# ALVI-Labs/frankenstein

Hardware: AMD Instinct MI355X
Metric: neural frames/sec (train fwd+bwd+AdamW, whole job) (higher is better)
Workload: dtype bf16; 1 GPU; brainformer-small (6L d=384 6x64 heads, N=6144 tokens) + 2-block perceiver, L1 head; fwd+bwd+clip+AdamW; per_gpu_batch=32, global_batch=32, frames_T=600, electrodes=256, parallelism=dp1, weights=random-init (seed 42)

## Files before the change

### frankenstein_amd/_lib.py

```python
from __future__ import annotations

import ctypes as C
from pathlib import Path

import os

LIB_PATH = Path(os.environ.get("FRANKEN_HIP_LIB") or Path(__file__).resolve().parent / "libfranken_hip.so")

FK_F32, FK_BF16 = 0, 1
MASK_NONE, MASK_CAUSAL, MASK_BLOCK_CAUSAL, MASK_PREFIX, MASK_KEYPAD, MASK_DENSE = 0, 1, 2, 3, 4, 5
NORM_LAYER, NORM_RMS = 0, 1
ATTN_Q_PRESCALED = 1
GEMV_GELU = 1
NT_RING2, NT_RING192, NT_RING128, NT_BIG, NT_GLDS4, NT_GLDS, NT_STAGED = range(7)
NT_LANE = 7
MLP_BWD_HIPCC, MLP_BWD_ASM = 0, 1
NT_ROUTE_F32 = -2
ATTN_FWD_GENERIC, ATTN_FWD_FEWQ, ATTN_FWD_PS, ATTN_FWD_ASM = range(4)
ATTN_DQ_GENERIC, ATTN_DQ_FEWQ, ATTN_DQ_PS, ATTN_DQ_ASM = range(4)
ATTN_DKDV_GENERIC, ATTN_DKDV_PS, ATTN_DKDV_ASM, ATTN_DKDVW_ASM = range(4)

_p, _i64, _int, _f32, _f64, _sz, _u32 = C.c_void_p, C.c_int64, C.c_int, C.c_float, C.c_double, C.c_size_t, C.c_uint32

SIGNATURES = {
    "fk_version": (_int, []),
    "fk_last_error": (C.c_char_p, []),
    "fk_gemm_nt": (_int, [_p, _i64, _p, _i64, _p, _i64, _i64, _i64, _i64, _p, _p, _i64, _i64, _int, _int, _p]),
    "fk_gemv_nt": (_int, [_p, _i64, _p, _i64, _p, _i64, _i64, _i64, _i64, _p, _p, _i64, _p, _p, _f32, _int, _int, _int, _p]),
    "fk_gemm_nt_rope": (_int, [_p, _i64, _p, _i64, _p, _i64, _i64, _i64, _i64, _p, _p, _i64, _i64, _i64, _i64, _i64, _i64, _i64, _int, _p]),
    "fk_gemm_nt_swiglu": (_int, [_p, _i64, _p, _i64, _p, _i64, _p, _i64, _i64, _i64, _i64, _int, _p]),
    "fk_gemm_nt_dswiglu": (_int, [_p, _i64, _p, _i64, _p, _i64, _p, _i64, _i64, _i64, _i64, _int, _p]),
    "fk_mlp_bwd_fused": (_int, [_p, _i64, _p, _i64, _p, _i64, _p, _i64, _p, _i64, _p, _i64, _i64, _i64, _i64, _int, _p]),
    "fk_gemm_nt_route": (_int, [_i64, _i64, _i64, _int, _int, _int, _int]),
    "fk_gemm_nt_rope_route": (_int, [_i64] * 6 + [_int] + [_i64] * 5 + [_int, _int]),
    "fk_gemm_nt_swiglu_route": (_int, [_i64] * 7 + [_int, _int]),
    "fk_mlp_bwd_fused_route": (_int, [_i64, _i64]),
    "fk_gemm_tn_route": (_int, [_i64, _i64, _i64, _int, _p, _p]),
    "fk_gemm_tn_workspace_bytes": (_sz, [_i64, _i64, _i64, _int]),
    "fk_gemm_tn": (_int, [_p, _i64, _p, _i64, _p, _i64, _i64, _i64, _i64, _int, _int, _p, _sz, _p]),
    "fk_gemm_tn_swiglu": (_int, [_p, _i64, _p, _i64, _p, _p, _i64, _i64, _i64, _i64, _int, _p, _sz, _p]),
    "fk_colsum_workspace_bytes": (_sz, [_i64, _i64]),
    "fk_colsum": (_int, [_p, _i64, _p, _i64, _i64, _int, _int, _p, _sz, _p]),
    "fk_attn_fwd": (_int, [_p, _p, _p, _p, _p] + [_i64] * 13 + [_int, _i64, _i64, _i64, _p, _p, _f32, _int, _int, _p]),
    "fk_attn_bwd": (_int, [_p] * 10 + [_i64] * 13 + [_int, _i64, _i64, _i64, _p, _p, _f32, _p, _i64, _i64, _int, _int, _p]),
    "fk_attn_fwd_dropout": (_int, [_p, _p, _p, _p, _p] + [_i64] * 13 + [_int, _i64, _i64, _i64, _p, _p, _f32, _int, _f32, _p, _u32, _int, _p]),
    "fk_attn_bwd_dropout": (_int, [_p] * 10 + [_i64] * 13 + [_int, _i64, _i64, _i64, _p, _p, _f32, _p, _i64, _i64, _int, _f32, _p, _u32, _int, _p]),
    "fk_attn_route": (_int, [_i64, _i64, _i64, _int, _int, _i64, _i64, _i64, _int, _int, _int, _p, _p, _p]),
    "fk_dropout": (_int, [_p, _p, _p, _i64, _f32, _p, _u32, _int, _p]),
    "fk_norm_fwd": (_int, [_p, _p, _p, _p, _p, _p, _i64, _i64, _f32, _int, _int, _p]),
    "fk_norm_bwd_workspace_bytes": (_sz, [_i64, _i64]),
    "fk_norm_bwd": (_int, [_p] * 9 + [_i64, _i64, _int, _int, _int, _p, _sz, _p]),
    "fk_rope": (_int, [_p, _i64, _i64, _i64, _i64, _i64, _p, _i64, _i64, _int, _int, _p]),
    "fk_patchify": (_int, [_p, _p, _i64, _i64, _i64, _i64, _i64, _int, _p]),
    "fk_swiglu_fwd": (_int, [_p, _p, _i64, _i64, _int, _p]),
    "fk_swiglu_bwd": (_int, [_p, _p, _p, _i64, _i64, _int, _p]),
    "fk_gelu_fwd": (_int, [_p, _p, _i64, _int, _p]),
    "fk_gelu_bwd": (_int, [_p, _p, _p, _i64, _int, _p]),
    "fk_cast_pack": (_int, [_p, _i64, _p, _i64, _i64, _i64, _int, _int, _p]),
    "fk_cast_pack_rows": (_int, [_p, _i64, _p, _i64, _i64, _i64, _int, _i64, _i64, _i64, _int, _p]),
    "fk_cast_pack_multi": (_int, [_p, _i64, _i64, _int, _p]),
    "fk_cast": (_int, [_p, _int, _p, _int, _i64, _p]),
    "fk_add": (_int, [_p, _p, _p, _i64, _int, _p]),
    "fk_gather_rows": (_int, [_p, _i64, _int, _p, _i64, _p, _i64, _int, _i64, _i64, _i64, _int, _p]),
# ... 141 lines not shown
```

### frankenstein_amd/csrc/gemm.hip

```cpp
#include <type_traits>

#include "fk_common.h"

namespace {

#ifndef FK_EPI_UNROLL
#define FK_EPI_UNROLL 1
#endif
#include "gemm_tile.h"

struct NtArgs {
  const void* A; const void* B; void* C;
  const void* bias; const void* res;
  int64_t lda, ldb, ldc, ldr, res_rows;
  int M, N, K, vec_epi;
  int mode;
  void* aux; int64_t ldaux;
  const float* rope_table; int64_t rope_bs; int rope_T, rope_off, rope_D, rope_cols;
  int rope_qcols; int64_t rope_qoff;
};

#ifndef FK_NT_STORES_GEMM
#define FK_NT_STORES_GEMM 1
#endif
// ... 1235 lines not shown
    for (; kt + TG_NS - 1 < nk; ++kt) step(Yes{}, Yes{}, Vm1{});
    if (kt + 2 < nk) { step(Yes{}, No{}, Vm1{}); ++kt; }
    if (kt + 1 < nk) step(Yes{}, No{}, Vm0{});
    step(No{}, No{}, Vm0{});
  }

  float* out = (p.nsplit > 1) ? p.ws + (int64_t)split * p.N1 * p.N2 : p.C;
  const int64_t ldo = (p.nsplit > 1) ? p.N2 : p.ldc;
  const bool accum = (p.nsplit == 1) && p.accumulate;
#pragma unroll
  for (int j = 0; j < NJ; ++j) {
    const int n = b0 + wn * WB + j * 32 + li;
#pragma unroll
    for (int i = 0; i < 3; ++i)
#pragma unroll
      for (int r = 0; r < 16; ++r) {
        const int m = a0 + wm * 96 + i * 32 + acc_row(r, lh);
        float* dst = out + (int64_t)m * ldo + n;
        *dst = accum ? (*dst + acc[i][j][r]) : acc[i][j][r];
      }
  }
}

template <bool IL>
__global__ __launch_bounds__(256) void reduce_slabs4_kernel(const float* ws, float* C, float* C1, int64_t ldc, int N1, int N2, int nsplit, int accumulate) {
  const int64_t total = (int64_t)N1 * N2, total4 = total >> 2;
  const int n2v = N2 >> 2;
  for (int64_t i = blockIdx.x * (int64_t)blockDim.x + threadIdx.x; i < total4; i += (int64_t)gridDim.x * blockDim.x) {
    const f32x4* src = reinterpret_cast<const f32x4*>(ws) + i;
    f32x4 s = {0.0f, 0.0f, 0.0f, 0.0f};
    int k = 0;
    for (; k + 8 <= nsplit; k += 8) {
      f32x4 v[8];
#pragma unroll
      for (int u = 0; u < 8; ++u) v[u] = src[(int64_t)(k + u) * total4];
#pragma unroll
      for (int u = 0; u < 8; ++u) s += v[u];
    }
    for (; k < nsplit; ++k) s += src[(int64_t)k * total4];
    int64_t r = i / n2v;
    float* base = C;
    if constexpr (IL) {
      if (r & 4) base = C1;
      r = (r >> 3) * 4 + (r & 3);
    }
    f32x4* dst = reinterpret_cast<f32x4*>(base + r * ldc + (i % n2v) * 4);
    if (accumulate) s += *dst;
    *dst = s;
  }
}
__global__ void reduce_slabs_kernel(const float* ws, float* C, int64_t ldc, int N1, int N2, int nsplit, int accumulate) {
  const int64_t total = (int64_t)N1 * N2;
  for (int64_t i = blockIdx.x * (int64_t)blockDim.x + threadIdx.x; i < total; i += (int64_t)gridDim.x * blockDim.x) {
    float s = 0.0f;
    for (int k = 0; k < nsplit; ++k) s += ws[k * total + i];
    float* dst = C + (i / N2) * ldc + (i % N2);
    *dst = accumulate ? (*dst + s) : s;
  }
}

template <typename T>
__global__ __launch_bounds__(256) void colsum_partial_kernel(const T* X, int64_t ld, float* part, int rows, int cols, int rows_per_blk) {
  constexpr int N = 16 / sizeof(T);
  __shared__ float red[256 * N];
  const int r0 = blockIdx.y * rows_per_blk, r1 = min(rows, r0 + rows_per_blk);
  const int cvt = (cols + N - 1) / N;
  {
    const int cv0 = blockIdx.x * 256;
    const int cvn = min(256, cvt - cv0), groups = 256 / cvn;
// ... 216 lines not shown

static int tn_plan(int64_t M, int64_t N1, int64_t N2, int dtype, int* nsplit, int64_t* rows_per_split) {
  const bool big = tn_big_ok(M, N1, N2, dtype);
  const int bkm = dtype == FK_BF16 ? 64 : 32;
  const int ns = big ? tn_big_splits(M, N1, N2) : tn_splits(M, N1, N2, bkm);
  if (nsplit) *nsplit = ns;
  if (rows_per_split) *rows_per_split = fk_cdiv(fk_cdiv(M, ns), bkm) * bkm;
  return big ? tn_big_tb(N1, N2) : 0;
}

int fk_gemm_tn_route(int64_t M, int64_t N1, int64_t N2, int dtype, int* nsplit, int64_t* rows_per_split) {
  FK_CHECK_ARG(dtype == FK_F32 || dtype == FK_BF16, "fk_gemm_tn_route: bad dtype %d", dtype);
  FK_CHECK_ARG(M > 0 && N1 > 0 && N2 > 0, "fk_gemm_tn_route: empty problem");
  return tn_plan(M, N1, N2, dtype, nsplit, rows_per_split);
}

size_t fk_gemm_tn_workspace_bytes(int64_t M, int64_t N1, int64_t N2, int dtype) {
  int ns;
  tn_plan(M, N1, N2, dtype, &ns, nullptr);
  return ns > 1 ? (size_t)ns * N1 * N2 * sizeof(float) : 0;
}

static int launch_tn(const void* A, int64_t lda, const void* B, int64_t ldb, float* C, float* C1, int64_t ldc, int64_t M, int64_t N1,
                     int64_t N2, int accumulate, int dtype, void* workspace, size_t workspace_bytes, void* stream) {
  FK_CHECK_ARG(dtype == FK_F32 || dtype == FK_BF16, "fk_gemm_tn: bad dtype %d", dtype);
  const int vec = dtype == FK_BF16 ? 8 : 4;
  FK_CHECK_ARG(M > 0 && N1 > 0 && N2 > 0, "fk_gemm_tn: empty problem");
  FK_CHECK_ARG(M < (1LL << 31) && N1 < (1LL << 31) && N2 < (1LL << 31), "fk_gemm_tn: dims must fit int32");
  FK_CHECK_ARG(N1 % vec == 0 && N2 % vec == 0 && lda % vec == 0 && ldb % vec == 0,
               "fk_gemm_tn: N1/N2/lda/ldb must be multiples of %d (N1=%lld N2=%lld)", vec, (long long)N1, (long long)N2);
  FK_CHECK_ARG(((uintptr_t)A & 15) == 0 && ((uintptr_t)B & 15) == 0, "fk_gemm_tn: A/B must be 16-byte aligned");
  int ns;
  int64_t rps;
  const int tb = tn_plan(M, N1, N2, dtype, &ns, &rps);
  const bool big = tb != 0;
  const size_t need = ns > 1 ? (size_t)ns * N1 * N2 * sizeof(float) : 0;
  FK_CHECK_ARG(workspace_bytes >= need && (need == 0 || workspace), "fk_gemm_tn: workspace too small (%zu < %zu)", workspace_bytes, need);
  if (C1)
    FK_CHECK_ARG(ns > 1 && N1 % 8 == 0 && N2 % 4 == 0 && ldc % 4 == 0 && (((uintptr_t)C | (uintptr_t)C1 | (uintptr_t)workspace) & 15) == 0,
                 "fk_gemm_tn_swiglu: needs a split plan (see fk_gemm_tn_route), N1 %% 8 == 0, N2 %% 4 == 0 and 16-byte aligned destinations");
  TnArgs p{A, B, C, (float*)workspace, lda, ldb, ldc, (int)M, (int)N1, (int)N2, (int)rps, ns, accumulate};
  dim3 grid((unsigned)(fk_cdiv(N1, BM) * fk_cdiv(N2, BN) * ns)), block(NTHREADS);
  hipStream_t s = (hipStream_t)stream;
  if (big) {
    dim3 bgrid((unsigned)((N1 / TG_A) * (N2 / tb) * ns));
    if (tb == 192) {
      constexpr int LDS192 = TG_NS * (TG_A_BYTES + TG_K * 512);
      fk_launch_lds<gemm_tn_big_kernel<192>>(bgrid, dim3(512), LDS192, s, p);
    } else {
      fk_launch_lds<gemm_tn_big_kernel<128>>(bgrid, dim3(512), TG_NS * TG_STAGE, s, p);
    }
  } else if (dtype == FK_BF16) hipLaunchKernelGGL((gemm_tn_kernel<bf16_t>), grid, block, 4 * TILE_BYTES, s, p);
  else hipLaunchKernelGGL((gemm_tn_kernel<float>), grid, block, 4 * TILE_BYTES, s, p);
  FK_CHECK_LAUNCH("fk_gemm_tn");
  if (ns > 1) {
    const int64_t total = N1 * N2;
    if (N2 % 4 == 0 && ldc % 4 == 0 && (((uintptr_t)C | (uintptr_t)workspace) & 15) == 0) {
      int nb = (int)fk_cdiv(total / 4, 256);
      if (nb > 2048) nb = 2048;
      if (C1) hipLaunchKernelGGL(reduce_slabs4_kernel<true>, dim3(nb), dim3(256), 0, s, (const float*)workspace, C, C1, ldc, (int)N1, (int)N2, ns, accumulate);
      else hipLaunchKernelGGL(reduce_slabs4_kernel<false>, dim3(nb), dim3(256), 0, s, (const float*)workspace, C, C1, ldc, (int)N1, (int)N2, ns, accumulate);
    } else {
      int nb = (int)fk_cdiv(total, 256);
      if (nb > 2048) nb = 2048;
      hipLaunchKernelGGL(reduce_slabs_kernel, dim3(nb), dim3(256), 0, s, (const float*)workspace, C, ldc, (int)N1, (int)N2, ns, accumulate);
    }
    FK_CHECK_LAUNCH("fk_gemm_tn(reduce)");
  }
  return FK_OK;
}

int fk_gemm_tn(const void* A, int64_t lda, const void* B, int64_t ldb, float* C, int64_t ldc, int64_t M, int64_t N1,
               int64_t N2, int accumulate, int dtype, void* workspace, size_t workspace_bytes, void* stream) {
  return launch_tn(A, lda, B, ldb, C, nullptr, ldc, M, N1, N2, accumulate, dtype, workspace, workspace_bytes, stream);
}

int fk_gemm_tn_swiglu(const void* A, int64_t lda, const void* B, int64_t ldb, float* d_up, float* d_gate, int64_t ldc, int64_t M,
                      int64_t H, int64_t N2, int dtype, void* workspace, size_t workspace_bytes, void* stream) {
  FK_CHECK_ARG(d_up && d_gate && H > 0 && H % 4 == 0, "fk_gemm_tn_swiglu: needs both destinations and H %% 4 == 0");
  return launch_tn(A, lda, B, ldb, d_up, d_gate, ldc, M, 2 * H, N2, 1, dtype, workspace, workspace_bytes, stream);
}

size_t fk_colsum_workspace_bytes(int64_t rows, int64_t cols) { return (size_t)colsum_blocks(rows) * cols * sizeof(float); }

int fk_colsum(const void* X, int64_t ld, float* out, int64_t rows, int64_t cols, int accumulate, int dtype,
              void* workspace, size_t workspace_bytes, void* stream) {
  FK_CHECK_ARG(dtype == FK_F32 || dtype == FK_BF16, "fk_colsum: bad dtype %d", dtype);
  FK_CHECK_ARG(rows > 0 && cols > 0 && rows < (1LL << 31) && cols < (1LL << 31), "fk_colsum: bad shape");
  const int nb = colsum_blocks(rows);
  FK_CHECK_ARG(workspace && workspace_bytes >= (size_t)nb * cols * sizeof(float), "fk_colsum: workspace too small");
  const int rpb = (int)fk_cdiv(rows, nb);
  hipStream_t s = (hipStream_t)stream;
  const int vec = dtype == FK_BF16 ? 8 : 4;
  if (cols % vec == 0 && ld % vec == 0 && ((uintptr_t)X & 15) == 0) {
    dim3 grid((unsigned)fk_cdiv(fk_cdiv(cols, vec), 256), (unsigned)nb), block(256);
    if (dtype == FK_BF16) hipLaunchKernelGGL(colsum_partial_kernel<bf16_t>, grid, block, 0, s, (const bf16_t*)X, ld, (float*)workspace, (int)rows, (int)cols, rpb);
    else hipLaunchKernelGGL(colsum_partial_kernel<float>, grid, block, 0, s, (const float*)X, ld, (float*)workspace, (int)rows, (int)cols, rpb);
  } else {
    dim3 grid((unsigned)fk_cdiv(cols, 256), (unsigned)nb), block(256);
    if (dtype == FK_BF16) hipLaunchKernelGGL(colsum_partial_scalar_kernel<bf16_t>, grid, block, 0, s, (const bf16_t*)X, ld, (float*)workspace, (int)rows, (int)cols, rpb);
    else hipLaunchKernelGGL(colsum_partial_scalar_kernel<float>, grid, block, 0, s, (const float*)X, ld, (float*)workspace, (int)rows, (int)cols, rpb);
  }
  FK_CHECK_LAUNCH("fk_colsum(partial)");
// ... 7 lines not shown
```

### frankenstein_amd/engine.py

```python
from __future__ import annotations

from typing import List, NamedTuple, Optional, Sequence, Tuple

import dataclasses
import math
import os
import weakref

import torch

from . import kernels as K
from .kernels import NO_MASK

Tensor = torch.Tensor

_COMPUTE_DTYPE = torch.bfloat16
_EPOCH = 0


def set_compute_dtype(dtype) -> None:
    global _COMPUTE_DTYPE
    if isinstance(dtype, str):
        dtype = {"bf16": torch.bfloat16, "bfloat16": torch.bfloat16, "fp32": torch.float32, "float32": torch.float32}[dtype]
    assert dtype in (torch.bfloat16, torch.float32)
# ... 8 lines not shown
    global _EPOCH
    _EPOCH += 1


_WGRAD_STREAM = None


def enable_wgrad_stream(on: bool = True):
    global _WGRAD_STREAM
    _WGRAD_STREAM = torch.cuda.Stream() if on else None
    return _WGRAD_STREAM


def wgrad_stream():
    return _WGRAD_STREAM


def _arena_grad(p: Tensor):
    g = p.grad
    return g if (g is not None and getattr(p, "_fk_arena", False) and g.is_contiguous()) else None


def wgrad_path(in_arena: Sequence[bool], swiglu_interleaved: bool = False, slab_ok: bool = False, adjacent: bool = False,
               requires_grad: Optional[Sequence[bool]] = None) -> str:
    if requires_grad is not None and not any(requires_grad):
        return "skip"
    if not all(in_arena):
        return "tensors"
    if swiglu_interleaved:
        return "swiglu_slab" if slab_ok else "swiglu_add"
    return "adjacent" if adjacent else "split_add"


def norm_bwd_path(gamma_in_arena: bool, has_beta: bool, beta_in_arena: bool) -> str:
    return "arena" if gamma_in_arena and (not has_beta or beta_in_arena) else "tensors"


def wgrad(a: Tensor, b: Tensor, params: Sequence[Tensor], swiglu_interleaved: bool = False):
    side = _WGRAD_STREAM
    grads = [_arena_grad(p) for p in params]
    in_arena = [g is not None for g in grads]
    first = wgrad_path(in_arena, swiglu_interleaved, requires_grad=[p.requires_grad for p in params])
    if first == "skip":
        return [None] * len(params)
    if first == "tensors":
        dw = K.gemm_tn(a, b)
        if swiglu_interleaved:
            return list(_deinterleave_rows(dw, params[0].shape[0]))
        return _split_rows(dw, params)
    if side is not None:
        side.wait_stream(torch.cuda.current_stream())
        a.record_stream(side)
        b.record_stream(side)
    with torch.cuda.stream(side if side is not None else torch.cuda.current_stream()):
        Kd = b.shape[1]
        adjacent = all(grads[i + 1].data_ptr() == grads[i].data_ptr() + grads[i].numel() * 4 for i in range(len(grads) - 1))
        path = wgrad_path(in_arena, swiglu_interleaved, swiglu_interleaved and K.gemm_tn_swiglu_ok(a, b, grads[0], grads[1]), adjacent)
        if path == "swiglu_slab":
            K.gemm_tn_swiglu_(a, b, grads[0], grads[1])
        elif path == "swiglu_add":
            dw = K.gemm_tn(a, b)
            H = params[0].shape[0]
            v = dw.view(H // 4, 8 * Kd)
            K.add2d_(grads[0].view(H // 4, 4 * Kd), v[:, :4 * Kd])
            K.add2d_(grads[1].view(H // 4, 4 * Kd), v[:, 4 * Kd:])
        elif path == "adjacent":
            n = sum(p.shape[0] for p in params)
            out = torch.as_strided(grads[0], (n, Kd), (Kd, 1))
            K.gemm_tn(a, b, out=out, accumulate=True)
        else:
            dw = K.gemm_tn(a, b)
            for g, part in zip(grads, _split_rows(dw, params)):
                K.add2d_(g.view(part.shape), part)
    return [None] * len(params)


def norm_bwd(dh: Tensor, x2: Tensor, ln_w: Tensor, ln_b: Optional[Tensor], mean: Tensor, rstd: Tensor, dres: Optional[Tensor] = None,
             kind: int = K.NORM_LAYER):
    gw = _arena_grad(ln_w)
    gb = _arena_grad(ln_b) if ln_b is not None else None
    if norm_bwd_path(gw is not None, ln_b is not None, gb is not None) == "arena":
        dx, _, _ = K.norm_bwd(dh, x2, ln_w.detach(), mean, rstd, dres=dres, kind=kind, want_beta=ln_b is not None,
                              dgamma=gw.view(-1), dbeta=None if gb is None else gb.view(-1), accumulate=True)
        return dx, None, None
    return K.norm_bwd(dh, x2, ln_w.detach(), mean, rstd, dres=dres, kind=kind, want_beta=ln_b is not None)


class _Shadow:
    __slots__ = ("stamp", "tensor", "jobs", "params", "dtype", "ptrs", "repack", "trained")

    def __init__(self):
        self.stamp, self.tensor, self.jobs, self.params, self.dtype, self.ptrs = None, None, [], (), None, ()
# ... 521 lines not shown
    def backward(ctx, dy):
        H, D, mask, eps = ctx.spec
        x, context, ln_w, qw, kw, vw, pw, h, mean, rstd, q, kv, o, lse = ctx.saved_tensors
        B, T, d = x.shape
        Nc, HD = context.shape[1], H * D
        x2, c2 = x.view(B * T, d), context.view(B * Nc, d)
        dy2 = dy.contiguous().view(B * T, d)
        do = K.gemm_nt(dy2, shadow([pw], transpose=True))
        (dpw,) = wgrad(dy2, o.view(B * T, HD), [pw])
        dkv = torch.empty_like(kv)
        dq = torch.empty_like(q)
        kv3, dkv3 = kv.view(B, Nc, 2 * HD), dkv.view(B, Nc, 2 * HD)
        K.attn_bwd(q.view(B, T, H, D), kv3[..., :HD].unflatten(-1, (H, D)), kv3[..., HD:].unflatten(-1, (H, D)), o,
                   do.view(B, T, H, D), lse, dq.view(B, T, H, D), dkv3[..., :HD].unflatten(-1, (H, D)),
                   dkv3[..., HD:].unflatten(-1, (H, D)), mask)
        dh = K.gemm_nt(dq, shadow([qw], transpose=True))
        (dqw,) = wgrad(dq, h, [qw])
        dctx = K.gemm_nt(dkv, shadow([kw, vw], transpose=True))
        dkw, dvw = wgrad(dkv, c2, [kw, vw])
        dx, dg, db = norm_bwd(dh, x2, ln_w, ctx.ln_b, mean, rstd, dres=dy2)
        return dx.view(B, T, d), dctx.view(B, Nc, d), dg, db, dqw, dkw, dvw, dpw, None


_MLP_BWD_FUSED = os.environ.get("FK_MLP_BWD_FUSED", "1") != "0"


def mlp_path(hidden: int, has_gate: bool, has_up_bias: bool) -> str:
    if not has_gate:
        return "gelu"
    return "swiglu_fused" if not has_up_bias and hidden % 8 == 0 else "swiglu"


def mlp_bwd_path(fused: bool, dtype, d: int, hidden: int, rows: int) -> str:
    if not fused:
        return "plain"
    if (_MLP_BWD_FUSED and dtype == torch.bfloat16 and d == 384 and hidden % 32 == 0 and rows >= 32768
            and rows * (2 * hidden) * 2 < 2 ** 32):
        return "one_launch"
    return "dswiglu"


class MlpBranch(torch.autograd.Function):

    @staticmethod
    def forward(ctx, x, ln_w, ln_b, up_w, up_b, gate_w, down_w, down_b, spec):
        return MlpBranch.run_forward(ctx, x, ln_w, ln_b, up_w, up_b, gate_w, down_w, down_b, spec, None)
# ... 845 lines not shown
```

### frankenstein_amd/kernels.py

```python
from __future__ import annotations

import ctypes
import math
from typing import Optional, Tuple

import torch

from . import _lib
from ._lib import FK_BF16, FK_F32, MASK_BLOCK_CAUSAL, MASK_CAUSAL, MASK_DENSE, MASK_KEYPAD, MASK_NONE, MASK_PREFIX, NORM_LAYER, NORM_RMS, ATTN_Q_PRESCALED, DAY_MAX_C, call, lib

Tensor = torch.Tensor


TIMERS = None
TIMER_PREFIX = None


class _timed:
    __slots__ = ("name", "ev")

    def __init__(self, name):
        self.name = name

    def __enter__(self):
        self.ev = None
        if TIMERS is not None and (TIMER_PREFIX is None or self.name.startswith(TIMER_PREFIX)):
            self.ev = (torch.cuda.Event(enable_timing=True), torch.cuda.Event(enable_timing=True))
# ... 216 lines not shown
        call("fk_gemm_tn", a.data_ptr(), a.stride(0), b.data_ptr(), b.stride(0), out.data_ptr(), out.stride(0), M, N1, N2,
             int(accumulate), fk_dtype(a), _ptr(ws), nb, _stream())
    return out


def gemm_tn_swiglu_ok(a: Tensor, b: Tensor, d_up: Tensor, d_gate: Tensor) -> bool:
    M, N1 = a.shape
    N2 = b.shape[1]
    return (gemm_tn_route(M, N1, N2, a.dtype)[1] > 1 and N1 % 8 == 0 and N2 % 4 == 0 and d_up.is_contiguous() and d_gate.is_contiguous()
            and d_up.data_ptr() % 16 == 0 and d_gate.data_ptr() % 16 == 0)


def gemm_tn_swiglu_(a: Tensor, b: Tensor, d_up: Tensor, d_gate: Tensor) -> None:
    assert a.dim() == 2 and b.dim() == 2 and a.shape[0] == b.shape[0] and a.dtype == b.dtype
    assert a.stride(1) == 1 and b.stride(1) == 1
    M, N1 = a.shape
    N2 = b.shape[1]
    for d in (d_up, d_gate):
        assert d.shape == (N1 // 2, N2) and d.dtype == torch.float32 and d.is_contiguous()
    ws, nb = _ws(lib().fk_gemm_tn_workspace_bytes(M, N1, N2, fk_dtype(a)), a.device)
    with _timed(f"gemm_tn_swiglu:{M}x{N1}x{N2}"):
        call("fk_gemm_tn_swiglu", a.data_ptr(), a.stride(0), b.data_ptr(), b.stride(0), d_up.data_ptr(), d_gate.data_ptr(), N2, M, N1 // 2,
             N2, fk_dtype(a), _ptr(ws), nb, _stream())


def colsum(x: Tensor, out: Optional[Tensor] = None, accumulate: bool = False) -> Tensor:
    assert x.dim() == 2 and x.stride(1) == 1
    rows, cols = x.shape
    if out is None:
        assert not accumulate
        out = torch.empty(cols, dtype=torch.float32, device=x.device)
    assert out.numel() == cols and out.dtype == torch.float32 and out.is_contiguous()
    ws, nb = _ws(lib().fk_colsum_workspace_bytes(rows, cols), x.device)
    call("fk_colsum", x.data_ptr(), x.stride(0), out.data_ptr(), rows, cols, int(accumulate), fk_dtype(x), _ptr(ws), nb,
         _stream())
    return out


class Mask:
    __slots__ = ("kind", "c", "q_off", "k_off", "limits", "qfirst")

    def __init__(self, kind: int = MASK_NONE, c: int = 0, q_off: int = 0, k_off: int = 0, limits=None, qfirst=None):
        self.kind, self.c, self.q_off, self.k_off, self.limits, self.qfirst = kind, c, q_off, k_off, limits, qfirst

    def sliced(self, n_full_q: int, n_full_k: int, t_q: int, t_k: int) -> "Mask":
        assert self.kind not in (MASK_PREFIX, MASK_KEYPAD, MASK_DENSE) or (n_full_q == t_q and n_full_k == t_k), "table masks cannot be sliced"
# ... 1388 lines not shown
```

### frankenstein_amd/models/brainformer.py

```python
from __future__ import annotations

from dataclasses import dataclass
from typing import Optional

import torch
import torch.nn as nn

from .. import engine as E
from .. import kernels as K
from ..kernels import MASK_BLOCK_CAUSAL, Mask, NO_MASK


class Serializable:
    pass


@dataclass
class MAEConfig(Serializable):
    window_size: int = 1024
    n_electrodes: int = 256
    patch_size: int = 48
    dim: int = 256
    n_layers: int = 4
    head_dim: int = 32
# ... 170 lines not shown
    def forward(self, x, attn_mask, rope, kv_cache=None):
        return self.branch(_prep(x), attn_mask, rope, None, False)


class CausalCrossAttention(nn.Module):
    def __init__(self, config, is_causal=True):
        super().__init__()
        assert config.n_heads == config.n_kv_heads, "n_heads should be equal n_kv_heads"
        self.n_heads = config.n_heads
        self.n_kv_heads = config.n_heads
        self.repeats = self.n_heads // self.n_kv_heads
        self.head_dim = config.head_dim
        self.qw = Linear(config.dim, config.head_dim * config.n_heads, bias=False)
        self.kw = Linear(config.dim, config.head_dim * config.n_kv_heads, bias=False)
        self.vw = Linear(config.dim, config.head_dim * config.n_kv_heads, bias=False)
        self.project = Linear(config.head_dim * config.n_heads, config.dim, bias=False)
        self.kv_cache = None

    def branch(self, x, context, attn_mask, ln: nn.LayerNorm):
        spec = (self.n_heads, self.head_dim, resolve_mask(attn_mask, x.shape[1], context.shape[1]), ln.eps)
        return E.CrossAttnBranch.apply(x, context, ln.weight, ln.bias, self.qw.weight, self.kw.weight,
                                       self.vw.weight, self.project.weight, spec)

    def forward(self, x, context, attn_mask=None, use_kv_cache=None):
        x, context = _prep(x), _prep(context)
        B, T, _ = x.shape
        H, D = self.n_heads, self.head_dim
        q = self.qw(x).view(B, T, H, D)
        k = self.kw(context).view(B, -1, H, D)
        v = self.vw(context).view(B, -1, H, D)
        o = _SDPA.apply(q, k, v, resolve_mask(attn_mask, T, context.shape[1]))
        return self.project(o.view(B, T, H * D))


class _SDPA(torch.autograd.Function):
    @staticmethod
    def forward(ctx, q, k, v, mask):
        o, lse = K.attn_fwd(q, k, v, mask)
        ctx.mask = mask
        ctx.save_for_backward(q, k, v, o, lse)
        return o

    @staticmethod
    def backward(ctx, do):
        q, k, v, o, lse = ctx.saved_tensors
        dq, dk, dv = torch.empty_like(q), torch.empty_like(k), torch.empty_like(v)
# ... 4 lines not shown
class Block(nn.Module):
    def __init__(self, config):
        super().__init__()
        self.ln_1 = LayerNorm(config.dim)
        self.attn = CausalSelfAttention(config)
        self.ln_2 = LayerNorm(config.dim)
        self.mlp = MLP(config)

    def forward(self, x, attn_mask=None, rope=None, kv_cache=False):
        x = _prep(x)
        x = self.attn.branch(x, attn_mask, rope, self.ln_1, True)
        return self.mlp.branch(x, self.ln_2, True)


class CrossBlock(nn.Module):
    def __init__(self, config):
        super().__init__()
        self.sa_block = Block(config)
        self.ln_1 = LayerNorm(config.dim)
        self.cross_attn = CausalCrossAttention(config)
        self.ln_2 = LayerNorm(config.dim)
        self.mlp = MLP(config)

    def forward(self, x, context, self_attn_mask=None, cross_attn_mask=None, sa_rope=None):
        x, context = _prep(x), _prep(context)
        x = self.cross_attn.branch(x, context, cross_attn_mask, self.ln_1)
        x = self.mlp.branch(x, self.ln_2, True)
        return self.sa_block(x, attn_mask=self_attn_mask, rope=sa_rope)


class DayAdapter(nn.Module):

    def __init__(self, n_days: int, n_channels: int):
        super().__init__()
        if n_days < 1 or not 1 <= n_channels <= K.DAY_MAX_C:
            raise ValueError(f"DayAdapter needs n_days >= 1 and 1 <= n_channels <= {K.DAY_MAX_C}, got {n_days}, {n_channels}")
        self.n_days, self.n_channels = n_days, n_channels
        self.delta = nn.Parameter(torch.zeros(n_days, n_channels, n_channels))
        self.bias = nn.Parameter(torch.zeros(n_days, n_channels))

    def tokens(self, x, date_info, P: int, ldp: int):
        return E.DayPatchify.apply(x, E.day_ids(date_info, x.shape[0], self.delta.device), self.delta, self.bias, P, ldp, False, True)

    def forward(self, x, date_info=None):
        B, T, C = x.shape
        day = E.day_ids(date_info, B, self.delta.device)
        return E.DayPatchify.apply(x, day, self.delta, self.bias, 1, 1, True).view(B, T, C)

    @torch.no_grad()
# ... 188 lines not shown
        loss = E.mse_loss(pred, target)
        if return_preds:
            with torch.no_grad():
                rec = K.cast(tok_p, torch.float32)
                K.scatter_rows_(rec, masked, pred.detach().float().contiguous())
                bm = torch.zeros_like(rec)
                K.scatter_rows_(bm, masked, torch.ones_like(pred, dtype=torch.float32))
            return loss, self.to_signal_shape(rec), self.to_signal_shape(bm)
        return (loss, None)


def _mae_get_sub_att_matrix(self, attn_mask, unmasked_indices):
    am = attn_mask.to(unmasked_indices.device)
    sub = am[unmasked_indices[:, :, None], unmasked_indices[:, None, :]]
    return sub[:, None]


MAE.get_sub_att_matrix = _mae_get_sub_att_matrix


class BrainFormer(nn.Module):
    config = Config
    head_name = 'to_motion'

    def __init__(self, config: Config):
        super().__init__()
        self.config = config
        self.encoder = Encoder(config.encoder)
        self.n_output_tokens = config.n_output_tokens
        self.learnable_queries = nn.Parameter(torch.zeros(1, config.n_output_tokens, config.dim))
        self.perceiver = nn.ModuleDict({
            'h': nn.ModuleList([CrossBlock(config) for _ in range(config.n_layers)]),
            'ln_f': LayerNorm(config.dim),
            self.head_name: Linear(config.dim, config.output_dim)})
        self.register_buffer('cross_attn_mask', None)
        self.register_buffer('self_attn_mask', None)
        self.precompute_rope_cash = build_complex_rope_cache(dim=config.head_dim, seq_len=config.n_output_tokens,
                                                             theta=config.rope_theta)
        print("Full HandFormer: number of parameters: %.2fM" % (self.get_num_params() / 1e6,))

    def get_num_params(self):
        return sum(p.numel() for p in self.parameters())

    @property
    def dtype(self) -> torch.dtype:
        return next(self.parameters()).dtype

    @property
    def device(self) -> torch.device:
        return next(self.parameters()).device

    @property
    def rope_cache(self) -> torch.Tensor:
        if self.precompute_rope_cash.device != self.device:
            self.precompute_rope_cash = self.precompute_rope_cash.to(device=self.device)
        return self.precompute_rope_cash

    def queries_out(self, x, date_info=None):
        b = x.shape[0]
        ctx = self.encoder(x, date_info=date_info)
        q = E.ExpandQueries.apply(self.learnable_queries, b)
        for cross_block in self.perceiver.h:
            q = cross_block(q, ctx, self.self_attn_mask, self.cross_attn_mask, sa_rope=self.rope_cache)
        return q

    def features(self, x, date_info=None):
        q = self.queries_out(x, date_info)
        head = self.perceiver[self.head_name]
        ln = self.perceiver.ln_f
        return E.NormLinear.apply(q, ln.weight, ln.bias, head.weight, head.bias, ln.eps, False)

    def forward(self, x, targets=None, date_info=None):
        pred = self.features(x, date_info)
        if targets is None:
            return None, pred
        return E.l1_loss(pred, targets), pred

    @torch.no_grad()
    def inference(self, myo, date_info):
        x = torch.from_numpy(myo)[None].to(self.device).float()
        pred = self.forward(x, targets=None, date_info=date_info)[1]
        return pred[0].float().cpu().numpy().T



def default_generation(model, emg, stride=8):
# ... 12 lines not shown
```

### include/franken_hip.h

```cpp
#ifndef FRANKEN_HIP_H
#define FRANKEN_HIP_H

#include <stddef.h>
#include <stdint.h>

#ifdef __cplusplus
extern "C" {
#endif

#define FK_VERSION 302

#define FK_OK 0
#define FK_EINVAL (-1)
#define FK_ELAUNCH (-2)
#define FK_EUNSUPPORTED (-3)

enum { FK_F32 = 0, FK_BF16 = 1 };
enum { FK_MASK_NONE = 0, FK_MASK_CAUSAL = 1, FK_MASK_BLOCK_CAUSAL = 2, FK_MASK_PREFIX = 3, FK_MASK_KEYPAD = 4, FK_MASK_DENSE = 5 };
enum { FK_ATTN_Q_PRESCALED = 1 };
enum { FK_NORM_LAYER = 0, FK_NORM_RMS = 1 };
enum { FK_ACT_SWIGLU = 0, FK_ACT_GELU = 1 };
enum { FK_GEMV_GELU = 1 };

int fk_version(void);
// ... 8 lines not shown
int fk_gemm_nt_rope(const void* A, int64_t lda, const void* B, int64_t ldb, void* C, int64_t ldc, int64_t M, int64_t N,
                    int64_t K, const void* bias, const float* table, int64_t table_bs, int64_t T, int64_t pos_off, int64_t D,
                    int64_t rot_cols, int64_t q_cols, int64_t q_table_off, int dtype, void* stream);
int fk_gemm_nt_swiglu(const void* A, int64_t lda, const void* W13, int64_t ldb, void* H13, int64_t ldh, void* G,
                      int64_t ldg, int64_t M, int64_t H, int64_t K, int dtype, void* stream);
int fk_gemm_nt_dswiglu(const void* dY, int64_t lda, const void* W2T, int64_t ldb, const void* H13, int64_t ldh, void* dH13,
                       int64_t lddh, int64_t M, int64_t H, int64_t K, int dtype, void* stream);
int fk_mlp_bwd_fused(const void* dY, int64_t lddy, const void* W2T, int64_t ldw2t, const void* H13, int64_t ldh, const void* W13T,
                     int64_t ldw13t, void* dH13, int64_t lddh, void* dX, int64_t lddx, int64_t M, int64_t H, int64_t D, int dtype,
                     void* stream);
enum { FK_NT_RING2 = 0, FK_NT_RING192 = 1, FK_NT_RING128 = 2, FK_NT_BIG = 3, FK_NT_GLDS4 = 4, FK_NT_GLDS = 5, FK_NT_STAGED = 6, FK_NT_LANE = 7 };
#define FK_NT_ROUTE_F32 (-2)
int fk_gemm_nt_route(int64_t M, int64_t N, int64_t K, int dtype, int vec_epi, int mode, int has_rope);
int fk_gemm_nt_rope_route(int64_t M, int64_t N, int64_t K, int64_t lda, int64_t ldb, int64_t ldc, int has_bias, int64_t T, int64_t pos_off,
                          int64_t D, int64_t rot_cols, int64_t q_cols, int align_ok, int dtype);
int fk_gemm_nt_swiglu_route(int64_t M, int64_t H, int64_t K, int64_t lda, int64_t ldb, int64_t ldh, int64_t ldg, int align_ok, int dtype);
enum { FK_MLP_BWD_HIPCC = 0, FK_MLP_BWD_ASM = 1 };
int fk_mlp_bwd_fused_route(int64_t M, int64_t lddh);
size_t fk_gemm_tn_workspace_bytes(int64_t M, int64_t N1, int64_t N2, int dtype);
int fk_gemm_tn(const void* A, int64_t lda, const void* B, int64_t ldb, float* C, int64_t ldc, int64_t M, int64_t N1,
               int64_t N2, int accumulate, int dtype, void* workspace, size_t workspace_bytes, void* stream);
int fk_gemm_tn_swiglu(const void* A, int64_t lda, const void* B, int64_t ldb, float* d_up, float* d_gate, int64_t ldc, int64_t M,
                      int64_t H, int64_t N2, int dtype, void* workspace, size_t workspace_bytes, void* stream);
int fk_gemm_tn_route(int64_t M, int64_t N1, int64_t N2, int dtype, int* nsplit, int64_t* rows_per_split);
size_t fk_colsum_workspace_bytes(int64_t rows, int64_t cols);
int fk_colsum(const void* X, int64_t ld, float* out, int64_t rows, int64_t cols, int accumulate, int dtype,
              void* workspace, size_t workspace_bytes, void* stream);

int fk_attn_fwd(const void* Q, const void* K, const void* V, void* O, float* LSE, int64_t B, int64_t H, int64_t Nq,
                int64_t Nk, int64_t D, int64_t q_bs, int64_t q_rs, int64_t k_bs, int64_t k_rs, int64_t v_bs,
                int64_t v_rs, int64_t o_bs, int64_t o_rs, int mask_kind, int64_t mask_c, int64_t q_off, int64_t k_off,
                const int32_t* limits, const int32_t* qfirst, float scale, int flags, int dtype, void* stream);
int fk_attn_bwd(const void* Q, const void* K, const void* V, const void* O, const void* dO, const float* LSE,
                void* dQ, void* dK, void* dV, float* delta_ws, int64_t B, int64_t H, int64_t Nq, int64_t Nk, int64_t D,
                int64_t q_bs, int64_t q_rs, int64_t k_bs, int64_t k_rs, int64_t v_bs, int64_t v_rs, int64_t o_bs,
                int64_t o_rs, int mask_kind, int64_t mask_c, int64_t q_off, int64_t k_off, const int32_t* limits,
                const int32_t* qfirst, float scale, const float* rope_table, int64_t rope_bs, int64_t rope_off, int flags,
                int dtype, void* stream);

int fk_attn_fwd_dropout(const void* Q, const void* K, const void* V, void* O, float* LSE, int64_t B, int64_t H, int64_t Nq,
                        int64_t Nk, int64_t D, int64_t q_bs, int64_t q_rs, int64_t k_bs, int64_t k_rs, int64_t v_bs,
                        int64_t v_rs, int64_t o_bs, int64_t o_rs, int mask_kind, int64_t mask_c, int64_t q_off, int64_t k_off,
                        const int32_t* limits, const int32_t* qfirst, float scale, int flags, float drop_p, const uint32_t* drop_seed,
                        uint32_t drop_site, int dtype, void* stream);
int fk_attn_bwd_dropout(const void* Q, const void* K, const void* V, const void* O, const void* dO, const float* LSE,
                        void* dQ, void* dK, void* dV, float* delta_ws, int64_t B, int64_t H, int64_t Nq, int64_t Nk, int64_t D,
// ... 285 lines not shown
```

Measured before the change: 399,000 frames/s.

## Batch perceiver cross-attention K/V projections across blocks with segmented weight-grad reduction

The K/V projections of the encoder context for every perceiver cross block are now computed in one GEMM, and their gradients are accumulated into one shared dK/dV buffer. The combined weight gradient is then computed with one split-K TN GEMM whose reduction kernel scatters rows into the separate per-parameter grad buffers. This replaces per-block context projections and per-block weight-grad GEMMs (or a split-then-add path) with fewer, larger launches. It adds a shared-buffer protocol between autograd functions and falls back to a zero-filled copy when the incoming gradients are not slices of the shared buffer.

Result: no change. 397,400 frames/s (-0.4%).

```diff
diff --git a/frankenstein_amd/_lib.py b/frankenstein_amd/_lib.py
--- a/frankenstein_amd/_lib.py
+++ b/frankenstein_amd/_lib.py
@@ -39,6 +39,7 @@
     "fk_gemm_tn_workspace_bytes": (_sz, [_i64, _i64, _i64, _int]),
     "fk_gemm_tn": (_int, [_p, _i64, _p, _i64, _p, _i64, _i64, _i64, _i64, _int, _int, _p, _sz, _p]),
     "fk_gemm_tn_swiglu": (_int, [_p, _i64, _p, _i64, _p, _p, _i64, _i64, _i64, _i64, _int, _p, _sz, _p]),
+    "fk_gemm_tn_segments": (_int, [_p, _i64, _p, _i64, _p, _p, _int, _i64, _i64, _i64, _int, _int, _p, _sz, _p]),
     "fk_colsum_workspace_bytes": (_sz, [_i64, _i64]),
     "fk_colsum": (_int, [_p, _i64, _p, _i64, _i64, _int, _int, _p, _sz, _p]),
     "fk_attn_fwd": (_int, [_p, _p, _p, _p, _p] + [_i64] * 13 + [_int, _i64, _i64, _i64, _p, _p, _f32, _int, _int, _p]),
diff --git a/frankenstein_amd/csrc/gemm.hip b/frankenstein_amd/csrc/gemm.hip
--- a/frankenstein_amd/csrc/gemm.hip
+++ b/frankenstein_amd/csrc/gemm.hip
@@ -1281,22 +1281,25 @@
   }
 }
 
+FK_DEV f32x4 slab_sum4(const f32x4* src, int64_t total4, int nsplit) {
+  f32x4 s = {0.0f, 0.0f, 0.0f, 0.0f};
+  int k = 0;
+  for (; k + 8 <= nsplit; k += 8) {
+    f32x4 v[8];
+#pragma unroll
+    for (int u = 0; u < 8; ++u) v[u] = src[(int64_t)(k + u) * total4];
+#pragma unroll
+    for (int u = 0; u < 8; ++u) s += v[u];
+  }
+  for (; k < nsplit; ++k) s += src[(int64_t)k * total4];
+  return s;
+}
 template <bool IL>
 __global__ __launch_bounds__(256) void reduce_slabs4_kernel(const float* ws, float* C, float* C1, int64_t ldc, int N1, int N2, int nsplit, int accumulate) {
   const int64_t total = (int64_t)N1 * N2, total4 = total >> 2;
   const int n2v = N2 >> 2;
   for (int64_t i = blockIdx.x * (int64_t)blockDim.x + threadIdx.x; i < total4; i += (int64_t)gridDim.x * blockDim.x) {
-    const f32x4* src = reinterpret_cast<const f32x4*>(ws) + i;
-    f32x4 s = {0.0f, 0.0f, 0.0f, 0.0f};
-    int k = 0;
-    for (; k + 8 <= nsplit; k += 8) {
-      f32x4 v[8];
-#pragma unroll
-      for (int u = 0; u < 8; ++u) v[u] = src[(int64_t)(k + u) * total4];
-#pragma unroll
-      for (int u = 0; u < 8; ++u) s += v[u];
-    }
-    for (; k < nsplit; ++k) s += src[(int64_t)k * total4];
+    f32x4 s = slab_sum4(reinterpret_cast<const f32x4*>(ws) + i, total4, nsplit);
     int64_t r = i / n2v;
     float* base = C;
     if constexpr (IL) {
@@ -1304,6 +1307,32 @@
       r = (r >> 3) * 4 + (r & 3);
     }
     f32x4* dst = reinterpret_cast<f32x4*>(base + r * ldc + (i % n2v) * 4);
+    if (accumulate) s += *dst;
+    *dst = s;
+  }
+}
+constexpr int TN_MAX_SEGS = 8;
+struct TnSegs {
+  float* dst[TN_MAX_SEGS];
+  int rows[TN_MAX_SEGS];
+  int n;
+};
+__global__ __launch_bounds__(256) void reduce_slabs4_segs_kernel(const float* ws, TnSegs sg, int N1, int N2, int nsplit, int accumulate) {
+  const int64_t total = (int64_t)N1 * N2, total4 = total >> 2;
+  const int n2v = N2 >> 2;
+  for (int64_t i = blockIdx.x * (int64_t)blockDim.x + threadIdx.x; i < total4; i += (int64_t)gridDim.x * blockDim.x) {
+    f32x4 s = slab_sum4(reinterpret_cast<const f32x4*>(ws) + i, total4, nsplit);
+    int r = (int)(i / n2v);
+    float* base = sg.dst[0];
+    int g = 0;
+#pragma unroll
+    for (int j = 0; j < TN_MAX_SEGS - 1; ++j)
+      if (g == j && j + 1 < sg.n && r >= sg.rows[j]) {
+        r -= sg.rows[j];
+        g = j + 1;
+        base = sg.dst[j + 1];
+      }
+    f32x4* dst = reinterpret_cast<f32x4*>(base + (int64_t)r * N2 + (i % n2v) * 4);
     if (accumulate) s += *dst;
     *dst = s;
   }
@@ -1566,7 +1595,7 @@
 }
 
 static int launch_tn(const void* A, int64_t lda, const void* B, int64_t ldb, float* C, float* C1, int64_t ldc, int64_t M, int64_t N1,
-                     int64_t N2, int accumulate, int dtype, void* workspace, size_t workspace_bytes, void* stream) {
+                     int64_t N2, int accumulate, int dtype, void* workspace, size_t workspace_bytes, void* stream, const TnSegs* segs = nullptr) {
   FK_CHECK_ARG(dtype == FK_F32 || dtype == FK_BF16, "fk_gemm_tn: bad dtype %d", dtype);
   const int vec = dtype == FK_BF16 ? 8 : 4;
   FK_CHECK_ARG(M > 0 && N1 > 0 && N2 > 0, "fk_gemm_tn: empty problem");
@@ -1583,6 +1612,9 @@
   if (C1)
     FK_CHECK_ARG(ns > 1 && N1 % 8 == 0 && N2 % 4 == 0 && ldc % 4 == 0 && (((uintptr_t)C | (uintptr_t)C1 | (uintptr_t)workspace) & 15) == 0,
                  "fk_gemm_tn_swiglu: needs a split plan (see fk_gemm_tn_route), N1 %% 8 == 0, N2 %% 4 == 0 and 16-byte aligned destinations");
+  if (segs)
+    FK_CHECK_ARG(ns > 1 && N2 % 4 == 0 && ((uintptr_t)workspace & 15) == 0,
+                 "fk_gemm_tn_segments: needs a split plan (see fk_gemm_tn_route), N2 %% 4 == 0 and a 16-byte aligned workspace");
   TnArgs p{A, B, C, (float*)workspace, lda, ldb, ldc, (int)M, (int)N1, (int)N2, (int)rps, ns, accumulate};
   dim3 grid((unsigned)(fk_cdiv(N1, BM) * fk_cdiv(N2, BN) * ns)), block(NTHREADS);
   hipStream_t s = (hipStream_t)stream;
@@ -1599,7 +1631,11 @@
   FK_CHECK_LAUNCH("fk_gemm_tn");
   if (ns > 1) {
     const int64_t total = N1 * N2;
-    if (N2 % 4 == 0 && ldc % 4 == 0 && (((uintptr_t)C | (uintptr_t)workspace) & 15) == 0) {
+    if (segs) {
+      int nb = (int)fk_cdiv(total / 4, 256);
+      if (nb > 2048) nb = 2048;
+      hipLaunchKernelGGL(reduce_slabs4_segs_kernel, dim3(nb), dim3(256), 0, s, (const float*)workspace, *segs, (int)N1, (int)N2, ns, accumulate);
+    } else if (N2 % 4 == 0 && ldc % 4 == 0 && (((uintptr_t)C | (uintptr_t)workspace) & 15) == 0) {
       int nb = (int)fk_cdiv(total / 4, 256);
       if (nb > 2048) nb = 2048;
       if (C1) hipLaunchKernelGGL(reduce_slabs4_kernel<true>, dim3(nb), dim3(256), 0, s, (const float*)workspace, C, C1, ldc, (int)N1, (int)N2, ns, accumulate);
@@ -1623,6 +1659,23 @@
                       int64_t H, int64_t N2, int dtype, void* workspace, size_t workspace_bytes, void* stream) {
   FK_CHECK_ARG(d_up && d_gate && H > 0 && H % 4 == 0, "fk_gemm_tn_swiglu: needs both destinations and H %% 4 == 0");
   return launch_tn(A, lda, B, ldb, d_up, d_gate, ldc, M, 2 * H, N2, 1, dtype, workspace, workspace_bytes, stream);
+}
+
+int fk_gemm_tn_segments(const void* A, int64_t lda, const void* B, int64_t ldb, float* const* dst, const int64_t* seg_rows, int nseg,
+                        int64_t M, int64_t N1, int64_t N2, int accumulate, int dtype, void* workspace, size_t workspace_bytes, void* stream) {
+  FK_CHECK_ARG(dst && seg_rows && nseg >= 1 && nseg <= TN_MAX_SEGS, "fk_gemm_tn_segments: needs 1 .. %d segments", TN_MAX_SEGS);
+  TnSegs sg{};
+  int64_t rows = 0;
+  for (int g = 0; g < nseg; ++g) {
+    FK_CHECK_ARG(dst[g] && ((uintptr_t)dst[g] & 15) == 0 && seg_rows[g] > 0 && seg_rows[g] < (1LL << 31),
+                 "fk_gemm_tn_segments: segment %d needs a 16-byte aligned destination and rows > 0", g);
+    sg.dst[g] = dst[g];
+    sg.rows[g] = (int)seg_rows[g];
+    rows += seg_rows[g];
+  }
+  sg.n = nseg;
+  FK_CHECK_ARG(rows == N1, "fk_gemm_tn_segments: the segments hold %lld rows, the product has %lld", (long long)rows, (long long)N1);
+  return launch_tn(A, lda, B, ldb, sg.dst[0], nullptr, N2, M, N1, N2, accumulate, dtype, workspace, workspace_bytes, stream, &sg);
 }
 
 size_t fk_colsum_workspace_bytes(int64_t rows, int64_t cols) { return (size_t)colsum_blocks(rows) * cols * sizeof(float); }
diff --git a/frankenstein_amd/engine.py b/frankenstein_amd/engine.py
--- a/frankenstein_amd/engine.py
+++ b/frankenstein_amd/engine.py
@@ -54,21 +54,23 @@
 
 
 def wgrad_path(in_arena: Sequence[bool], swiglu_interleaved: bool = False, slab_ok: bool = False, adjacent: bool = False,
-               requires_grad: Optional[Sequence[bool]] = None) -> str:
+               requires_grad: Optional[Sequence[bool]] = None, segments_ok: bool = False) -> str:
     if requires_grad is not None and not any(requires_grad):
         return "skip"
     if not all(in_arena):
         return "tensors"
     if swiglu_interleaved:
         return "swiglu_slab" if slab_ok else "swiglu_add"
-    return "adjacent" if adjacent else "split_add"
+    if adjacent:
+        return "adjacent"
+    return "segments" if segments_ok else "split_add"
 
 
 def norm_bwd_path(gamma_in_arena: bool, has_beta: bool, beta_in_arena: bool) -> str:
     return "arena" if gamma_in_arena and (not has_beta or beta_in_arena) else "tensors"
 
 
-def wgrad(a: Tensor, b: Tensor, params: Sequence[Tensor], swiglu_interleaved: bool = False):
+def wgrad(a: Tensor, b: Tensor, params: Sequence[Tensor], swiglu_interleaved: bool = False, segments: bool = False):
     side = _WGRAD_STREAM
     grads = [_arena_grad(p) for p in params]
     in_arena = [g is not None for g in grads]
@@ -87,7 +89,10 @@
     with torch.cuda.stream(side if side is not None else torch.cuda.current_stream()):
         Kd = b.shape[1]
         adjacent = all(grads[i + 1].data_ptr() == grads[i].data_ptr() + grads[i].numel() * 4 for i in range(len(grads) - 1))
-        path = wgrad_path(in_arena, swiglu_interleaved, swiglu_interleaved and K.gemm_tn_swiglu_ok(a, b, grads[0], grads[1]), adjacent)
+        segs_ok = (segments and not swiglu_interleaved and not adjacent and
+                   K.gemm_tn_segments_ok(a.shape[0], a.shape[1], Kd, a.dtype, len(grads), all(g.data_ptr() % 16 == 0 for g in grads)))
+        path = wgrad_path(in_arena, swiglu_interleaved, swiglu_interleaved and K.gemm_tn_swiglu_ok(a, b, grads[0], grads[1]), adjacent,
+                          segments_ok=segs_ok)
         if path == "swiglu_slab":
             K.gemm_tn_swiglu_(a, b, grads[0], grads[1])
         elif path == "swiglu_add":
@@ -100,6 +105,8 @@
             n = sum(p.shape[0] for p in params)
             out = torch.as_strided(grads[0], (n, Kd), (Kd, 1))
             K.gemm_tn(a, b, out=out, accumulate=True)
+        elif path == "segments":
+            K.gemm_tn_segments_(a, b, [g.view(p.shape[0], Kd) for g, p in zip(grads, params)], accumulate=True)
         else:
             dw = K.gemm_tn(a, b)
             for g, part in zip(grads, _split_rows(dw, params)):
@@ -667,6 +674,102 @@
         return dx.view(B, T, d), dctx.view(B, Nc, d), dg, db, dqw, dkw, dvw, dpw, None
 
 
+class SharedKV:
+    __slots__ = ("shape", "dtype", "device", "width", "dkv")
+
+    def __init__(self, kv: Tensor, width: int):
+        self.shape, self.dtype, self.device, self.width, self.dkv = tuple(kv.shape), kv.dtype, kv.device, width, None
+
+    def grad_slice(self, index: int) -> Tensor:
+        if self.dkv is None:
+            self.dkv = torch.empty(self.shape, dtype=self.dtype, device=self.device)
+        return self.dkv[:, index * self.width:(index + 1) * self.width]
+
+    def is_slice(self, g: Optional[Tensor], index: int) -> bool:
+        buf = self.dkv
+        return (g is not None and buf is not None and g.dtype == buf.dtype and tuple(g.shape) == (buf.shape[0], self.width)
+                and g.stride() == buf.stride() and g.data_ptr() == buf.data_ptr() + index * self.width * buf.element_size())
+
+
+class ContextKV(torch.autograd.Function):
+
+    @staticmethod
+    def forward(ctx, context, shared_box, *kv_w):
+        B, Nc, d = context.shape
+        L = len(kv_w) // 2
+        kv = K.gemm_nt(context.view(B * Nc, d), shadow(list(kv_w)))
+        width = kv.shape[1] // L
+        assert all(w.shape[0] * 2 == width for w in kv_w), "the cross blocks of one perceiver have one K / V width"
+        shared = shared_box[0] = SharedKV(kv, width)
+        ctx.shared = shared
+        ctx.set_materialize_grads(False)
+        ctx.save_for_backward(context, *kv_w)
+        return tuple(kv[:, l * width:(l + 1) * width] for l in range(L))
+
+    @staticmethod
+    def backward(ctx, *grads):
+        context, *kv_w = ctx.saved_tensors
+        shared = ctx.shared
+        B, Nc, d = context.shape
+        if all(shared.is_slice(g, l) for l, g in enumerate(grads)):
+            dkv = shared.dkv
+        else:
+            dkv = torch.zeros(shared.shape, dtype=shared.dtype, device=shared.device)
+            for l, g in enumerate(grads):
+                if g is not None:
+                    K.copy2d(g if g.stride(1) == 1 else g.contiguous(), dkv[:, l * shared.width:(l + 1) * shared.width])
+        shared.dkv = None
+        dctx = K.gemm_nt(dkv, shadow(kv_w, transpose=True)).view(B, Nc, d) if ctx.needs_input_grad[0] else None
+        dws = wgrad(dkv, context.view(B * Nc, d), kv_w, segments=True)
+        return (dctx, None, *dws)
+
+
+def context_kv(context: Tensor, kv_w: Sequence[Tensor]):
+    box = [None]
+    slices = ContextKV.apply(context, box, *kv_w)
+    return [(s, box[0], l) for l, s in enumerate(slices)]
+
+
+class CrossAttnBranchKV(torch.autograd.Function):
+
+    @staticmethod
+    def forward(ctx, x, kv, ln_w, ln_b, qw, pw, spec, shared, index):
+        H, D, mask, eps = spec
+        B, T, d = x.shape
+        HD = H * D
+        x2 = x.view(B * T, d)
+        h, mean, rstd = K.norm_fwd(x2, ln_w.detach(), ln_b.detach(), eps)
+        ctx.ln_b = ln_b
+        q = K.gemm_nt(h, shadow([qw]))
+        kv3 = kv.view(B, -1, 2 * HD)
+        o, lse = K.attn_fwd(q.view(B, T, H, D), kv3[..., :HD].unflatten(-1, (H, D)), kv3[..., HD:].unflatten(-1, (H, D)), mask)
+        y = K.gemm_nt(o.view(B * T, HD), shadow([pw]), residual=x2)
+        ctx.spec, ctx.shared, ctx.index = spec, shared, index
+        ctx.save_for_backward(x, kv, ln_w, qw, pw, h, mean, rstd, q, o, lse)
+        return y.view(B, T, d)
+
+    @staticmethod
+    def backward(ctx, dy):
+        H, D, mask, eps = ctx.spec
+        x, kv, ln_w, qw, pw, h, mean, rstd, q, o, lse = ctx.saved_tensors
+        B, T, d = x.shape
+        HD = H * D
+        x2 = x.view(B * T, d)
+        dy2 = dy.contiguous().view(B * T, d)
+        do = K.gemm_nt(dy2, shadow([pw], transpose=True))
+        (dpw,) = wgrad(dy2, o.view(B * T, HD), [pw])
+        dkv = ctx.shared.grad_slice(ctx.index)
+        dq = torch.empty_like(q)
+        kv3, dkv3 = kv.view(B, -1, 2 * HD), dkv.view(B, -1, 2 * HD)
+        K.attn_bwd(q.view(B, T, H, D), kv3[..., :HD].unflatten(-1, (H, D)), kv3[..., HD:].unflatten(-1, (H, D)), o,
+                   do.view(B, T, H, D), lse, dq.view(B, T, H, D), dkv3[..., :HD].unflatten(-1, (H, D)),
+                   dkv3[..., HD:].unflatten(-1, (H, D)), mask)
+        dh = K.gemm_nt(dq, shadow([qw], transpose=True))
+        (dqw,) = wgrad(dq, h, [qw])
+        dx, dg, db = norm_bwd(dh, x2, ln_w, ctx.ln_b, mean, rstd, dres=dy2)
+        return dx.view(B, T, d), dkv, dg, db, dqw, dpw, None, None, None
+
+
 _MLP_BWD_FUSED = os.environ.get("FK_MLP_BWD_FUSED", "1") != "0"
 
 
diff --git a/frankenstein_amd/kernels.py b/frankenstein_amd/kernels.py
--- a/frankenstein_amd/kernels.py
+++ b/frankenstein_amd/kernels.py
@@ -2,7 +2,7 @@
 
 import ctypes
 import math
-from typing import Optional, Tuple
+from typing import Optional, Sequence, Tuple
 
 import torch
 
@@ -265,6 +265,30 @@
     with _timed(f"gemm_tn_swiglu:{M}x{N1}x{N2}"):
         call("fk_gemm_tn_swiglu", a.data_ptr(), a.stride(0), b.data_ptr(), b.stride(0), d_up.data_ptr(), d_gate.data_ptr(), N2, M, N1 // 2,
              N2, fk_dtype(a), _ptr(ws), nb, _stream())
+
+
+TN_MAX_SEGMENTS = 8
+
+
+def gemm_tn_segments_ok(M: int, N1: int, N2: int, dtype, n_segments: int, aligned: bool = True) -> bool:
+    return 1 <= n_segments <= TN_MAX_SEGMENTS and aligned and N2 % 4 == 0 and gemm_tn_route(M, N1, N2, dtype)[1] > 1
+
+
+def gemm_tn_segments_(a: Tensor, b: Tensor, dsts: Sequence[Tensor], accumulate: bool = True) -> None:
+    import ctypes
+    assert a.dim() == 2 and b.dim() == 2 and a.shape[0] == b.shape[0] and a.dtype == b.dtype
+    assert a.stride(1) == 1 and b.stride(1) == 1
+    M, N1 = a.shape
+    N2 = b.shape[1]
+    for d in dsts:
+        assert d.dim() == 2 and d.shape[1] == N2 and d.dtype == torch.float32 and d.is_contiguous()
+    n = len(dsts)
+    ptrs = (ctypes.c_void_p * n)(*[d.data_ptr() for d in dsts])
+    rows = (ctypes.c_int64 * n)(*[d.shape[0] for d in dsts])
+    ws, nb = _ws(lib().fk_gemm_tn_workspace_bytes(M, N1, N2, fk_dtype(a)), a.device)
+    with _timed(f"gemm_tn_segments:{M}x{N1}x{N2}"):
+        call("fk_gemm_tn_segments", a.data_ptr(), a.stride(0), b.data_ptr(), b.stride(0), ctypes.addressof(ptrs), ctypes.addressof(rows), n,
+             M, N1, N2, int(accumulate), fk_dtype(a), _ptr(ws), nb, _stream())
 
 
 def colsum(x: Tensor, out: Optional[Tensor] = None, accumulate: bool = False) -> Tensor:
diff --git a/frankenstein_amd/models/brainformer.py b/frankenstein_amd/models/brainformer.py
--- a/frankenstein_amd/models/brainformer.py
+++ b/frankenstein_amd/models/brainformer.py
@@ -216,6 +216,10 @@
         return E.CrossAttnBranch.apply(x, context, ln.weight, ln.bias, self.qw.weight, self.kw.weight,
                                        self.vw.weight, self.project.weight, spec)
 
+    def branch_kv(self, x, kv, n_ctx: int, attn_mask, ln: nn.LayerNorm):
+        spec = (self.n_heads, self.head_dim, resolve_mask(attn_mask, x.shape[1], n_ctx), ln.eps)
+        return E.CrossAttnBranchKV.apply(x, kv[0], ln.weight, ln.bias, self.qw.weight, self.project.weight, spec, kv[1], kv[2])
+
     def forward(self, x, context, attn_mask=None, use_kv_cache=None):
         x, context = _prep(x), _prep(context)
         B, T, _ = x.shape
@@ -266,9 +270,12 @@
         self.ln_2 = LayerNorm(config.dim)
         self.mlp = MLP(config)
 
-    def forward(self, x, context, self_attn_mask=None, cross_attn_mask=None, sa_rope=None):
-        x, context = _prep(x), _prep(context)
-        x = self.cross_attn.branch(x, context, cross_attn_mask, self.ln_1)
+    def forward(self, x, context, self_attn_mask=None, cross_attn_mask=None, sa_rope=None, kv=None):
+        x = _prep(x)
+        if kv is not None:
+            x = self.cross_attn.branch_kv(x, kv, context.shape[1], cross_attn_mask, self.ln_1)
+        else:
+            x = self.cross_attn.branch(x, _prep(context), cross_attn_mask, self.ln_1)
         x = self.mlp.branch(x, self.ln_2, True)
         return self.sa_block(x, attn_mask=self_attn_mask, rope=sa_rope)
 
@@ -503,6 +510,7 @@
 class BrainFormer(nn.Module):
     config = Config
     head_name = 'to_motion'
+    share_context_kv = True
 
     def __init__(self, config: Config):
         super().__init__()
@@ -541,8 +549,13 @@
         b = x.shape[0]
         ctx = self.encoder(x, date_info=date_info)
         q = E.ExpandQueries.apply(self.learnable_queries, b)
-        for cross_block in self.perceiver.h:
-            q = cross_block(q, ctx, self.self_attn_mask, self.cross_attn_mask, sa_rope=self.rope_cache)
+        blocks = list(self.perceiver.h)
+        kvs = [None] * len(blocks)
+        if len(blocks) > 1 and self.share_context_kv:
+            ctx = _prep(ctx)
+            kvs = E.context_kv(ctx, [w for blk in blocks for w in (blk.cross_attn.kw.weight, blk.cross_attn.vw.weight)])
+        for cross_block, kv in zip(blocks, kvs):
+            q = cross_block(q, ctx, self.self_attn_mask, self.cross_attn_mask, sa_rope=self.rope_cache, kv=kv)
         return q
 
     def features(self, x, date_info=None):
diff --git a/include/franken_hip.h b/include/franken_hip.h
--- a/include/franken_hip.h
+++ b/include/franken_hip.h
@@ -54,6 +54,8 @@
                int64_t N2, int accumulate, int dtype, void* workspace, size_t workspace_bytes, void* stream);
 int fk_gemm_tn_swiglu(const void* A, int64_t lda, const void* B, int64_t ldb, float* d_up, float* d_gate, int64_t ldc, int64_t M,
                       int64_t H, int64_t N2, int dtype, void* workspace, size_t workspace_bytes, void* stream);
+int fk_gemm_tn_segments(const void* A, int64_t lda, const void* B, int64_t ldb, float* const* dst, const int64_t* seg_rows, int nseg,
+                        int64_t M, int64_t N1, int64_t N2, int accumulate, int dtype, void* workspace, size_t workspace_bytes, void* stream);
 int fk_gemm_tn_route(int64_t M, int64_t N1, int64_t N2, int dtype, int* nsplit, int64_t* rows_per_split);
 size_t fk_colsum_workspace_bytes(int64_t rows, int64_t cols);
 int fk_colsum(const void* X, int64_t ld, float* out, int64_t rows, int64_t cols, int accumulate, int dtype,
```
